# jdeschut/tunempc

Hardware: AMD Instinct MI355X
Metric: stage-Hessian convexifications/sec at (nx+nu)=32, p=64 (higher is better)
Workload: dtype f64

## Files before the change

### include/tunempc_hip.h

```cpp
#ifndef TUNEMPC_HIP_H
#define TUNEMPC_HIP_H

#include <stdint.h>

#ifdef __cplusplus
extern "C" {
#endif

#define TMPC_OK 0
#define TMPC_E_ARG (-1)
#define TMPC_E_UNSUPPORTED (-2)
#define TMPC_E_NOMEM (-3)
#define TMPC_E_HIP (-4)
#define TMPC_E_NODEVICE (-5)
#define TMPC_E_NOCONV (-6)

#define TMPC_STATUS_OPTIMAL 0
#define TMPC_STATUS_FEASIBLE 1
#define TMPC_STATUS_INFEASIBLE 2

#define TMPC_FLAG_NO_MFMA 1
#define TMPC_FLAG_PROFILE 2
#define TMPC_FLAG_FAST_EXIT 4

// ... 15 lines not shown
int tmpc_destroy(tmpc_handle* h);
int tmpc_get_chunk(tmpc_handle* h);

int tmpc_set_options(tmpc_handle* h, double tol, double center_tol, int max_iter, int center_iter, int flags);

#define TMPC_TUNE_CHORD_STEP 1
#define TMPC_TUNE_SMALL_BLOCKS 2
#define TMPC_TUNE_EIG_PRETEST 3
#define TMPC_TUNE_FUSE_FWD 4
#define TMPC_TUNE_GRAPH 5
#define TMPC_TUNE_PERSISTENT 7
#define TMPC_TUNE_LOWP_SWITCH 8
#define TMPC_LOWP_SWITCH_DEFAULT 1e-5
#define TMPC_TUNE_LOWP_TRSM 9
#define TMPC_TUNE_TRSM_PAIR 10
int tmpc_set_tuning(tmpc_handle* h, int key, double value);
int tmpc_create_ex(tmpc_handle** out, int chunk, int p, int nx, int mb, int ng, int nc, int step3, int lanes);

int tmpc_set_tight(tmpc_handle* h, int enable, double tight_tol);

int tmpc_convexify_batch_host(tmpc_handle* h, int nb, const double* A, const double* B, const double* H,
                              double* Hc, double* dHc, double* P, double* alpha, double* beta, double* kappa,
                              int32_t* status, int32_t* iters, double* info);
int tmpc_convexify_batch_device(tmpc_handle* h, int nb, const double* dA, const double* dB, const double* dH,
                                double* dHc_out, double* ddHc_out, double* dP_out, double* d_alpha, double* d_beta,
                                double* d_kappa, int32_t* d_status, int32_t* d_iters, double* d_info, void* stream);

int tmpc_convexify_eq_batch_host(tmpc_handle* h, int nb, const double* A, const double* B, const double* H, const double* G,
                                 double* Hc, double* dHc, double* P, double* Fg, double* alpha, double* beta, double* kappa,
                                 int32_t* status, int32_t* iters, double* info);
// ... 167 lines not shown
```

### include/tunempc_hip_debug.h

```cpp
#ifndef TUNEMPC_HIP_DEBUG_H
#define TUNEMPC_HIP_DEBUG_H

#include "tunempc_hip.h"

#ifdef __cplusplus
extern "C" {
#endif

#define TMPC_DEBUG_FLAG_STOP_ASSEMBLED 8
#define TMPC_DEBUG_FLAG_NO_LIFT 16
#define TMPC_DEBUG_FLAG_NO_DMA 32
#define TMPC_DEBUG_FLAG_GENERIC_STAGE 64

int tmpc_debug_gemm_nt(tmpc_handle* h, double* C, const double* A, const double* B, int M, int N, int K, int mode, int lower);

int tmpc_debug_block_solve(tmpc_handle* h, int p, int d, const double* D, const double* Ccpl, const double* rhs, double* x, int32_t* nshift);

#define TMPC_DEBUG_FACTOR_PASS1 1
#define TMPC_DEBUG_FACTOR_FUSE_FWD1 2
#define TMPC_DEBUG_FACTOR_LOWP_TRSM 4
#define TMPC_DEBUG_FACTOR_DD 8
typedef struct {
  const double *D, *Ccpl, *Dlo, *Clo, *rhs;
  const int32_t *list, *lowp;
  double *oD, *oO, *oF, *oDdiag, *oX;
  float* oO32;
  double *oDl, *oOl, *oFl, *oXl;
  int32_t *nshift, *dims, *orient;
} tmpc_debug_factor_io;
int tmpc_debug_block_factor(tmpc_handle* h, int nb, int p, int d, int count, int mode, const tmpc_debug_factor_io* io);
long long tmpc_debug_last_trsm_pairs(void);

int tmpc_debug_cr_schedule(int p, int32_t* out, int cap);

int tmpc_debug_get_multipliers(tmpc_handle* h, int nb, int nr, double* phi, double* z, double* dphi, double* dz);

int tmpc_debug_get_array(tmpc_handle* h, int which, uint64_t offset, uint64_t count, double* out);

int tmpc_debug_set_stop_iteration(tmpc_handle* h, int k);

int tmpc_debug_min_eig(tmpc_handle* h, int nmat, int n, const double* W, double* out);
int tmpc_debug_min_eig_lane(tmpc_handle* h, int nmat, int n, const double* W, double* out);

int tmpc_debug_factor_bench(tmpc_handle* h, int nb, int p, int d, int reps, double* ms_out2);

#ifdef __cplusplus
// ... 4 lines not shown
```

### tunempc_amd/_lib.py

```python
import ctypes as C
import os

import numpy as np

_HERE = os.path.dirname(os.path.abspath(__file__))
_LIB = None

INFO_STRIDE = 16
FLAG_NO_MFMA = 1
FLAG_PROFILE = 2
FLAG_FAST_EXIT = 4
STATUS_NAMES = {0: 'Optimal', 1: 'Feasible', 2: 'Infeasible'}

ARROW_LD = 32
EXPORTS = [
    'tmpc_device_count', 'tmpc_workspace_bytes', 'tmpc_workspace_bytes_eq', 'tmpc_workspace_bytes_con',
    'tmpc_create', 'tmpc_create_eq', 'tmpc_create_con', 'tmpc_destroy', 'tmpc_get_chunk', 'tmpc_set_options', 'tmpc_set_tight', 'tmpc_set_tuning', 'tmpc_create_ex',
    'tmpc_convexify_batch_host', 'tmpc_convexify_batch_device', 'tmpc_convexify_eq_batch_host', 'tmpc_convexify_step2_batch_host',
    'tmpc_convexify_con_batch_device', 'tmpc_workspace_bytes_step3', 'tmpc_create_step3', 'tmpc_convexify_step3_batch_host', 'tmpc_workspace_bytes_step3_con', 'tmpc_create_step3_con', 'tmpc_convexify_step3_con_batch_host', 'tmpc_convexify_step3_batch_device', 'tmpc_convexify_step3_con_batch_device', 'tmpc_supplement_batch_host', 'tmpc_supplement_terms_batch_host',
    'tmpc_tracking_reference_host', 'tmpc_eig_scan_host', 'tmpc_get_profile', 'tmpc_get_trace', 'tmpc_get_dual_host', 'tmpc_get_dual_con_host', 'tmpc_pack_sensitivities_host', 'tmpc_eig_clip_host',
    'tmpc_periodic_lqr_batch_host', 'tmpc_periodic_lqr_batch_device', 'tmpc_periodic_lqr_rows_batch_host', 'tmpc_periodic_lqr_rows_batch_device',
    'tmpc_periodic_lqr_ctg_batch_host', 'tmpc_periodic_lqr_ctg_batch_device', 'tmpc_horizon_lqr_batch_host', 'tmpc_horizon_lqr_batch_device',
    'tmpc_closed_loop_batch_host', 'tmpc_closed_loop_batch_device', 'tmpc_mpc_qp_batch_host', 'tmpc_mpc_qp_batch_device',
    'tmpc_mpc_qp_soft_batch_host', 'tmpc_mpc_qp_soft_batch_device', 'tmpc_mpc_qp_eq_batch_host', 'tmpc_mpc_qp_eq_batch_device',
    'tmpc_mpc_qp_aff_batch_host', 'tmpc_mpc_qp_aff_batch_device', 'tmpc_mpc_qp_quad_batch_host', 'tmpc_mpc_qp_quad_batch_device',
    'tmpc_mpc_qp_warm_batch_host', 'tmpc_mpc_qp_warm_batch_device',
    'tmpc_last_error', 'tmpc_version',
]
DEBUG_EXPORTS = [
    'tmpc_debug_gemm_nt', 'tmpc_debug_block_solve', 'tmpc_debug_cr_schedule', 'tmpc_debug_get_multipliers', 'tmpc_debug_get_array',
    'tmpc_debug_min_eig', 'tmpc_debug_min_eig_lane', 'tmpc_debug_factor_bench', 'tmpc_debug_block_factor',
    'tmpc_debug_last_trsm_pairs', 'tmpc_debug_set_stop_iteration',
]
FLAG_DEBUG_NO_DMA = 32
FACTOR_PASS1, FACTOR_FUSE_FWD1, FACTOR_LOWP_TRSM, FACTOR_DD = 1, 2, 4, 8


class _FactorIO(C.Structure):
    _fields_ = ([(n, C.POINTER(C.c_double)) for n in ('D', 'Ccpl', 'Dlo', 'Clo', 'rhs')] + [(n, C.POINTER(C.c_int32)) for n in ('list', 'lowp')] +
                [(n, C.POINTER(C.c_double)) for n in ('oD', 'oO', 'oF', 'oDdiag', 'oX')] + [('oO32', C.POINTER(C.c_float))] +
                [(n, C.POINTER(C.c_double)) for n in ('oDl', 'oOl', 'oFl', 'oXl')] + [(n, C.POINTER(C.c_int32)) for n in ('nshift', 'dims', 'orient')])


def library_path():
    return os.environ.get('TMPC_LIB') or os.path.join(_HERE, 'lib', 'libtunempc_hip.so')


# ... 131 lines not shown
    lib.tmpc_debug_gemm_nt.argtypes = [vp, dp, dp, dp, C.c_int, C.c_int, C.c_int, C.c_int, C.c_int]
    lib.tmpc_debug_block_solve.restype = C.c_int
    lib.tmpc_debug_block_solve.argtypes = [vp, C.c_int, C.c_int, dp, dp, dp, dp, ip]
    lib.tmpc_supplement_terms_batch_host.restype = C.c_int
    lib.tmpc_supplement_terms_batch_host.argtypes = [vp, C.c_int, dp, dp, dp, C.c_int, dp, dp, dp, dp]
    lib.tmpc_tracking_reference_host.restype = C.c_int
    lib.tmpc_tracking_reference_host.argtypes = [vp, C.c_int, dp, dp, dp, C.c_double, dp, dp, ip]
    lib.tmpc_debug_cr_schedule.restype = C.c_int
    lib.tmpc_debug_cr_schedule.argtypes = [C.c_int, ip, C.c_int]
    lib.tmpc_debug_block_factor.restype = C.c_int
    lib.tmpc_debug_block_factor.argtypes = [vp, C.c_int, C.c_int, C.c_int, C.c_int, C.c_int, C.POINTER(_FactorIO)]
    lib.tmpc_debug_factor_bench.restype = C.c_int
    lib.tmpc_debug_factor_bench.argtypes = [vp, C.c_int, C.c_int, C.c_int, C.c_int, dp]
    lib.tmpc_debug_last_trsm_pairs.restype = C.c_longlong
    lib.tmpc_debug_last_trsm_pairs.argtypes = []
    lib.tmpc_debug_min_eig.restype = C.c_int
    lib.tmpc_debug_min_eig.argtypes = [vp, C.c_int, C.c_int, dp, dp]
    lib.tmpc_debug_min_eig_lane.restype = C.c_int
    lib.tmpc_debug_min_eig_lane.argtypes = [vp, C.c_int, C.c_int, dp, dp]
    lib.tmpc_last_error.restype = C.c_char_p
    lib.tmpc_version.restype = C.c_char_p
    _LIB = lib
    return lib


def _dptr(a):
    return a.ctypes.data_as(C.POINTER(C.c_double)) if a is not None else None


def _iptr(a):
# ... 34 lines not shown
            _check(self.lib, self.lib.tmpc_create_step3_con(C.byref(self._h), int(chunk), self.p, self.nx, self.mb, self.ng, self.nc), 'tmpc_create_step3_con')
        elif self.step3:
            _check(self.lib, self.lib.tmpc_create_step3(C.byref(self._h), int(chunk), self.p, self.nx, self.mb), 'tmpc_create_step3')
        else:
            _check(self.lib, self.lib.tmpc_create_con(C.byref(self._h), int(chunk), self.p, self.nx, self.mb, self.ng, self.nc), 'tmpc_create_con')
        self.chunk = int(self.lib.tmpc_get_chunk(self._h))
        self.flags = int(flags)
        self.set_options(tol, center_tol, max_iter, center_iter, flags)

    def set_options(self, tol=None, center_tol=None, max_iter=None, center_iter=None, flags=None):
        if flags is not None:
            self.flags = int(flags)
        _check(self.lib, self.lib.tmpc_set_options(self._h, float(tol or 0.0), float(center_tol or 0.0),
                                                   int(max_iter or 0), int(center_iter or 0), self.flags), 'tmpc_set_options')

    def set_tuning(self, chord_step=None, small_blocks=None, eig_pretest=None, fuse_fwd=None, graph=None, persistent=None, lowp_switch=None, lowp_trsm=None, trsm_pair=None):
        for key, v in ((1, chord_step), (2, small_blocks), (3, eig_pretest), (4, fuse_fwd), (5, graph), (7, persistent), (8, lowp_switch), (9, lowp_trsm), (10, trsm_pair)):
            if v is not None:
                _check(self.lib, self.lib.tmpc_set_tuning(self._h, key, float(v)), 'tmpc_set_tuning')

    def set_tight(self, enable=True, tight_tol=None):
        _check(self.lib, self.lib.tmpc_set_tight(self._h, 1 if enable else 0, float(tight_tol or 0.0)), 'tmpc_set_tight')

    def close(self):
        if getattr(self, '_h', None) is not None and self._h.value:
            self.lib.tmpc_destroy(self._h)
            self._h = C.c_void_p()

    def __del__(self):
        try:
            self.close()
        except Exception:
# ... 283 lines not shown
        if Hc.shape[-2:] != (n, n) or q.shape != Hc.shape[:-1] or wref.shape != q.shape:
            raise ValueError('tracking_reference: expected Hc [..., %d, %d] and q, wref [..., %d]' % (n, n, n))
        ns = int(np.prod(Hc.shape[:-2], dtype=np.int64))
        W = np.empty_like(Hc); yref = np.empty_like(q); info = np.zeros(Hc.shape[:-2], dtype=np.int32)
        _check(self.lib, self.lib.tmpc_tracking_reference_host(self._h, ns, _dptr(Hc), _dptr(q), _dptr(wref), float(ts), _dptr(W), _dptr(yref),
                                                              info.ctypes.data_as(C.POINTER(C.c_int32))), 'tmpc_tracking_reference_host')
        return W, yref, info

    def debug_factor_bench(self, nb, p, d, reps=3):
        out = np.zeros(2)
        _check(self.lib, self.lib.tmpc_debug_factor_bench(self._h, nb, p, d, reps, _dptr(out)), 'tmpc_debug_factor_bench')
        return out

    def debug_last_trsm_pairs(self):
        return int(self.lib.tmpc_debug_last_trsm_pairs())

    def debug_block_solve(self, D, Ccpl, rhs):
        D = np.ascontiguousarray(D, dtype=np.float64); Ccpl = np.ascontiguousarray(Ccpl, dtype=np.float64)
        rhs = np.ascontiguousarray(rhs, dtype=np.float64)
        p, d, _ = D.shape
        x = np.empty((p, d)); ns = np.zeros(1, np.int32)
        _check(self.lib, self.lib.tmpc_debug_block_solve(self._h, p, d, _dptr(D), _dptr(Ccpl), _dptr(rhs), _dptr(x), _iptr(ns)), 'tmpc_debug_block_solve')
        return x, int(ns[0])

    def debug_block_factor(self, D, Ccpl, rhs, plist=None, lowp=None, pass1=False, fuse_fwd1=False, lowp_trsm=False, dd=False, Dlo=None, Clo=None):
        f64 = lambda a: None if a is None else np.ascontiguousarray(a, dtype=np.float64)
        D, Ccpl, rhs, Dlo, Clo = f64(D), f64(Ccpl), f64(rhs), f64(Dlo), f64(Clo)
        nb, p, d, _ = D.shape
        nc = 3 if pass1 else 1
        if Ccpl.shape != D.shape or rhs.shape != ((nb, p, d, 3) if pass1 else (nb, p, d)):
# ... 430 lines not shown
```

### tunempc_amd/csrc/tmpc_api.hip

```cpp
#include <hip/hip_runtime.h>
#include <stdio.h>
#include <stdlib.h>
#include <new>
#include <string.h>
#include <algorithm>
#include <chrono>
#include <thread>
#include <mutex>
#include <condition_variable>
#include <functional>
#include <unistd.h>
#include <vector>

#include <string>
#include <unordered_map>

#include "../../include/tunempc_hip.h"
#include "../../include/tunempc_hip_debug.h"
#include "tmpc_common.h"
#include "tmpc_small.h"
#include "tmpc_stage.h"
#include "tmpc_schur.h"
#include "tmpc_factor.h"
#include "tmpc_cr.h"
// ... 96 lines not shown
struct tmpc_handle {
  Dims dm;
  int chunk;
  int nlanes;
  Opts opt;
  int flags;
  int stop_it;
  Lane lane[MAXL];
  void* slab;
  size_t slab_bytes;
  hipEvent_t ev_in;
  int device;
  CrSched sched;
  int* d_sched;
  int rs, mt;
  int tune_small, tune_pretest, tune_fuse, tune_graph, tune_persist, tune_lowp_trsm, tune_trsm_pair;
  void* dd_slab;
  size_t dd_bytes;
  int tight;
  double tight_tol;
};

static int cr_upload(const CrSched& sc, int** out) {
  std::vector<int> flat(sc.elim);
  flat.insert(flat.end(), sc.upd.begin(), sc.upd.end());
  flat.insert(flat.end(), sc.orient.begin(), sc.orient.end());
  *out = nullptr;
  if (hipMalloc(out, flat.size() * sizeof(int)) != hipSuccess) return TMPC_E_NOMEM;
  if (hipMemcpy(*out, flat.data(), flat.size() * sizeof(int), hipMemcpyHostToDevice) != hipSuccess) { hipFree(*out); *out = nullptr; return TMPC_E_HIP; }
  return TMPC_OK;
}
// ... 274 lines not shown
  const int m0 = 64 * tm, n0 = 64 * tn;
  const int Mt = M - m0 < 64 ? M - m0 : 64, Nt = N - n0 < 64 ? N - n0 : 64;
  const double* A0 = A + (size_t)m0 * K; const double* B0 = B + (size_t)n0 * K;
  if (k1 > 0 && k1 < K && 2 * k1 == K)
    wg_tile_dma<UPD_DMA_DEPTH>(C + (size_t)m0 * N + n0, N, A0, B0, A0 + k1, B0 + k1, K, Mt, Nt, k1, mode, (lower && tm == tn) ? 0 : GM_NOTRI, blockIdx.x, lds);
  else
    wg_tile_dma<UPD_DMA_DEPTH>(C + (size_t)m0 * N + n0, N, A0, B0, nullptr, nullptr, K, Mt, Nt, K, mode, (lower && tm == tn) ? 0 : GM_NOTRI, blockIdx.x, lds);
}
static size_t slots_bytes(int s) { return (size_t)s * MS * sizeof(double); }
template <int PART> static size_t schur_lds(const Dims& dm) {
  if (!schur_in_lds(dm)) return (size_t)dm.d * sizeof(unsigned) + 64;
 return (size_t)sch_rec<PART>() * dm.nx * dm.nx * sizeof(double) + (size_t)dm.d * sizeof(unsigned) + 64; }
static size_t factor_lds() { return (size_t)FACT_LDS_DOUBLES * sizeof(double); }
static size_t solve_lds(const Dims& dm) { return (size_t)cr_solve_lds_doubles(dm.dp) * sizeof(double); }

static int set_lds_attrs(int device) {
  static bool done[64] = {false};
  if (device >= 0 && device < 64 && done[device]) return TMPC_OK;
  const int big = 160 * 1024;
  HIPCHK(hipFuncSetAttribute((const void*)k_stage_pre<256>, hipFuncAttributeMaxDynamicSharedMemorySize, big - 4096));
  HIPCHK(hipFuncSetAttribute((const void*)k_stage_rhs<256>, hipFuncAttributeMaxDynamicSharedMemorySize, big - 4096));
  HIPCHK(hipFuncSetAttribute((const void*)k_stage_dir<256>, hipFuncAttributeMaxDynamicSharedMemorySize, big - 4096));
  HIPCHK(hipFuncSetAttribute((const void*)k_final_stage, hipFuncAttributeMaxDynamicSharedMemorySize, big));
  HIPCHK(hipFuncSetAttribute((const void*)k_schur<0>, hipFuncAttributeMaxDynamicSharedMemorySize, big));
  HIPCHK(hipFuncSetAttribute((const void*)k_schur<1>, hipFuncAttributeMaxDynamicSharedMemorySize, big));
  HIPCHK(hipFuncSetAttribute((const void*)k_cr_potrf<true>, hipFuncAttributeMaxDynamicSharedMemorySize, big));
  HIPCHK(hipFuncSetAttribute((const void*)k_cr_potrf<false>, hipFuncAttributeMaxDynamicSharedMemorySize, big));
  HIPCHK(hipFuncSetAttribute((const void*)k_cr_trsm<true, 2>, hipFuncAttributeMaxDynamicSharedMemorySize, big));
  HIPCHK(hipFuncSetAttribute((const void*)k_cr_trsm<false, 2>, hipFuncAttributeMaxDynamicSharedMemorySize, big));
  HIPCHK(hipFuncSetAttribute((const void*)k_cr_trsm_dma, hipFuncAttributeMaxDynamicSharedMemorySize, big));
  HIPCHK(hipFuncSetAttribute((const void*)k_cr_trsm_dma_f32, hipFuncAttributeMaxDynamicSharedMemorySize, big));
  HIPCHK(hipFuncSetAttribute((const void*)k_cr_potrf_dma, hipFuncAttributeMaxDynamicSharedMemorySize, big));
  HIPCHK(hipFuncSetAttribute((const void*)k_cr_update<true, 2>, hipFuncAttributeMaxDynamicSharedMemorySize, big));
  HIPCHK(hipFuncSetAttribute((const void*)k_cr_update<false, 2>, hipFuncAttributeMaxDynamicSharedMemorySize, big));
  HIPCHK(hipFuncSetAttribute((const void*)k_cr_fwd_diag, hipFuncAttributeMaxDynamicSharedMemorySize, big));
  HIPCHK(hipFuncSetAttribute((const void*)k_cr_fwd_off, hipFuncAttributeMaxDynamicSharedMemorySize, big));
  HIPCHK(hipFuncSetAttribute((const void*)k_cr_bwd, hipFuncAttributeMaxDynamicSharedMemorySize, big));
  HIPCHK(hipFuncSetAttribute((const void*)k_cr_small_solve, hipFuncAttributeMaxDynamicSharedMemorySize, big));
  HIPCHK(hipFuncSetAttribute((const void*)k_cr_small_factor, hipFuncAttributeMaxDynamicSharedMemorySize, big));
  HIPCHK(hipFuncSetAttribute((const void*)k_ipm_small, hipFuncAttributeMaxDynamicSharedMemorySize, big));
// ... 265 lines not shown
    }
  }
  auto ipm_loop = [&](const Opts& o, bool ddm, int cap) -> int {
  while (active > 0 && it < cap) {
    const int BP = active * dm.p;
    hipGraphExec_t gexec = nullptr;
    std::string gkey;
    bool capturing = false;
    struct CaptureGuard {
      hipStream_t st; bool* on;
      ~CaptureGuard() { if (*on) { hipGraph_t g_ = nullptr; (void)hipStreamEndCapture(st, &g_); if (g_) hipGraphDestroy(g_); (void)hipGetLastError(); } }
    } capture_guard{st, &capturing};
    int nkev = 0;
    if (use_graph && !ddm) {
      gkey.assign((const char*)&w, sizeof(WS)); gkey.append((const char*)&dm, sizeof(Dims)); gkey.append((const char*)&o, sizeof(Opts));
      const int ks[6] = {active, nfac, nb, reg_max, (int)h->flags, h->tune_pretest | (h->tune_fuse << 1) | (h->tune_small << 2)};
      gkey.append((const char*)ks, sizeof(ks));
      if (!ln->graphs) ln->graphs = new std::unordered_map<std::string, hipGraphExec_t>();
      auto f = ln->graphs->find(gkey);
      if (f == ln->graphs->end()) {
        if (ln->graphs->size() >= 256) { for (auto& kv : *ln->graphs) if (kv.second) hipGraphExecDestroy(kv.second); ln->graphs->clear(); }
        (*ln->graphs)[gkey] = nullptr;
      } else if (f->second) gexec = f->second;
      else if (hipStreamBeginCapture(st, hipStreamCaptureModeThreadLocal) == hipSuccess) capturing = true;
    }
    if (!gexec) {
    if (prof) HIPCHK(hipEventRecord(ln->ev[0], st));
    if (big) hipLaunchKernelGGL(kb_stage_pre, dim3(BP), dim3(256), 0, st, w, dm);
    else TMPC_STAGE_LAUNCH(k_stage_pre, slots_bytes(PRE_SLOTS), st, w, dm);
    if (eq) {
      const bool bigr = dm.nr > NRS;
      if (big && bigr) hipLaunchKernelGGL((k_phi_pre<true, true>), dim3(BP), dim3(64), (size_t)phi_pre_lds(true, true) * sizeof(double), st, w, dm, 1);
      else if (big) hipLaunchKernelGGL((k_phi_pre<true, false>), dim3(BP), dim3(64), (size_t)phi_pre_lds(true, false) * sizeof(double), st, w, dm, 1);
      else if (bigr) hipLaunchKernelGGL((k_phi_pre<false, true>), dim3(BP), dim3(64), (size_t)phi_pre_lds(false, true) * sizeof(double), st, w, dm, 1);
      else hipLaunchKernelGGL((k_phi_pre<false, false>), dim3(BP), dim3(64), (size_t)phi_pre_lds(false, false) * sizeof(double), st, w, dm, 1);
    }
    if (t3) hipLaunchKernelGGL(k_t3_pre, dim3(BP), dim3(64), t3_lds, st, w, dm);
    hipLaunchKernelGGL(k_ctrl_a, dim3(active), dim3(64), 0, st, w, dm, o);
    if (prof) HIPCHK(hipEventRecord(ln->ev[1], st));
    if (ddm) {
      if (nfac > 0) {
        hipLaunchKernelGGL(k_dd_images, dim3(nfac * dm.p), dim3(256), dd_stage_lds(dm, DD_IMG_SLOTS), st, wf, dm);
        dd_schur_launch(wf, dm, nfac * dm.p, st);
      }
    } else if (nfac > 0) {
      if (schur_in_lds(dm)) {
        hipLaunchKernelGGL(k_schur<0>, dim3(nfac * dm.p), dim3(SCH_NT), schur_lds<0>(dm), st, wf, dm);
        hipLaunchKernelGGL(k_schur<1>, dim3(nfac * dm.p), dim3(SCH_NT), schur_lds<1>(dm), st, wf, dm);
      } else {
        hipLaunchKernelGGL((k_schur<0, true>), dim3(nfac * dm.p), dim3(SCH_NT), schur_lds<0>(dm), st, wf, dm);
        hipLaunchKernelGGL((k_schur<1, true>), dim3(nfac * dm.p), dim3(SCH_NT), schur_lds<1>(dm), st, wf, dm);
      }
    }
    if (eq && nfac > 0 && ddm) hipLaunchKernelGGL(k_dd_aug_fill, dim3(nfac * dm.p), dim3(256), (size_t)dd_aug_lds_doubles(dm.nr, dm.n, dm.nx) * sizeof(double), st, wf, dm, 0);
    else if (eq && nfac > 0) hipLaunchKernelGGL(k_aug_fill, dim3(nfac * dm.p), dim3(64), 0, st, wf, dm);
    if (t3 && nfac > 0 && big) hipLaunchKernelGGL(k_t3_schur<true>, dim3(nfac * dm.p), dim3(256), t3_schur_lds, st, wf, dm);
    else if (t3 && nfac > 0) hipLaunchKernelGGL(k_t3_schur<false>, dim3(nfac * dm.p), dim3(256), t3_schur_lds, st, wf, dm);
    if (t3 && eq && nfac > 0) hipLaunchKernelGGL(k_t3_cross, dim3(nfac * dm.p), dim3(64), 0, st, wf, dm);
    if ((h->flags & TMPC_DEBUG_FLAG_STOP_ASSEMBLED) && it + 1 >= h->stop_it) {
      if (big) hipLaunchKernelGGL(kb_stage_rhs, dim3(BP), dim3(256), 0, st, w, dm, 1);
      else TMPC_STAGE_LAUNCH(k_stage_rhs, slots_bytes(RHS_SLOTS), st, w, dm, 1);
      if (t3) hipLaunchKernelGGL(k_t3_rhs, dim3(BP), dim3(64), t3_lds, st, w, dm, 1);
      hipLaunchKernelGGL(k_gather, dim3(BP), dim3(64), 0, st, w, dm, 1);
      if (t3) hipLaunchKernelGGL(k_t3_gather, dim3(BP), dim3(64), 0, st, w, dm, 1);
      HIPCHK(hipStreamSynchronize(st));
// ... 238 lines not shown
  }
  tmpc_handle* h = new (std::nothrow) tmpc_handle();
  if (!h) return TMPC_E_NOMEM;
  h->slab = nullptr; h->d_sched = nullptr; h->ev_in = nullptr; h->dd_slab = nullptr; h->dd_bytes = 0; h->tight = 0; h->tight_tol = 0x1p-37;
  if (hipGetDevice(&h->device) != hipSuccess) { delete h; return TMPC_E_HIP; }
  int nl = (make_dims(1, p, nx, mb, ng, nc, step3).dp <= 64 && chunk >= 2) ? 2 : 1;
  if (lanes >= 1) nl = std::min(lanes, MAXL);
  nl = std::max(1, std::min(nl, chunk));
  h->nlanes = nl;
  const int cap = (chunk + nl - 1) / nl;
  h->chunk = cap * nl;
  h->dm = make_dims(cap, p, nx, mb, ng, nc, step3);
  h->sched = cr_build(p);
  h->rs = 0; h->mt = 0;
  h->tune_small = 1; h->tune_pretest = 1; h->tune_fuse = 1; h->tune_graph = 1; h->tune_persist = 1; h->tune_lowp_trsm = 1; h->tune_trsm_pair = 1;
  h->opt.tol = 0x1p-25; h->opt.center_tol = 1e-9; h->opt.max_iter = 50; h->opt.center_iter = 12;
  h->opt.fast_exit = 0;
  h->opt.lowp_switch = TMPC_LOWP_SWITCH_DEFAULT;
  h->opt.chord_step = 10.0;
  h->flags = 0; h->stop_it = 1;
  WS tmp;
  const size_t lane_bytes = carve(tmp, h->dm, nullptr, nullptr);
  h->slab_bytes = lane_bytes * nl;
  if (hipMalloc(&h->slab, h->slab_bytes) != hipSuccess) {
    snprintf(g_err, sizeof(g_err), "hipMalloc(%zu bytes) failed", h->slab_bytes);
    delete h;
    return TMPC_E_NOMEM;
  }
  int rc = cr_upload(h->sched, &h->d_sched);
  bool ok = (rc == TMPC_OK) && hipEventCreateWithFlags(&h->ev_in, hipEventDisableTiming) == hipSuccess;
// ... 52 lines not shown
}


int tmpc_set_tuning(tmpc_handle* h, int key, double value) {
  if (!h) return TMPC_E_ARG;
  switch (key) {
    case TMPC_TUNE_CHORD_STEP: if (!(value >= 0.0)) return TMPC_E_ARG; h->opt.chord_step = value; return TMPC_OK;
    case TMPC_TUNE_LOWP_SWITCH: if (!(value >= 0.0)) return TMPC_E_ARG; h->opt.lowp_switch = value; return TMPC_OK;
    case TMPC_TUNE_SMALL_BLOCKS: h->tune_small = value != 0.0; return TMPC_OK;
    case TMPC_TUNE_EIG_PRETEST: h->tune_pretest = value != 0.0; return TMPC_OK;
    case TMPC_TUNE_FUSE_FWD: h->tune_fuse = value != 0.0; return TMPC_OK;
    case TMPC_TUNE_GRAPH: h->tune_graph = value != 0.0; return TMPC_OK;
    case TMPC_TUNE_PERSISTENT: if (!(value >= 0.0 && value <= 2.0)) return TMPC_E_ARG; h->tune_persist = (int)value; return TMPC_OK;
    case TMPC_TUNE_LOWP_TRSM: h->tune_lowp_trsm = value != 0.0; return TMPC_OK;
    case TMPC_TUNE_TRSM_PAIR: h->tune_trsm_pair = value != 0.0; return TMPC_OK;
    default: snprintf(g_err, sizeof(g_err), "tmpc_set_tuning: unknown key %d", key); return TMPC_E_ARG;
  }
}

int tmpc_set_tight(tmpc_handle* h, int enable, double tight_tol) {
  if (!h) return TMPC_E_ARG;
  if (!enable) { h->tight = 0; return TMPC_OK; }
  if (h->dm.nT > 0) { snprintf(g_err, sizeof(g_err), "tmpc_set_tight: Steps 1 and 2 only (no Step 3 handles)"); return TMPC_E_UNSUPPORTED; }
  if (h->dm.nr > 0 && (size_t)dd_aug_lds_doubles(h->dm.nr, h->dm.n, h->dm.nx) * sizeof(double) > 160 * 1024) {
    snprintf(g_err, sizeof(g_err), "tmpc_set_tight: %d rows per stage at nx = %d, nx + mb = %d: their double-double vectors do not fit the LDS (rows * (2 n + 2 nx) <= 4040)", h->dm.nr, h->dm.nx, h->dm.n);
    return TMPC_E_UNSUPPORTED;
  }
  if ((size_t)dd_solve_lds_doubles(h->dm.dp) * sizeof(double) > 160 * 1024) {
    snprintf(g_err, sizeof(g_err), "tmpc_set_tight: Schur blocks of %d do not fit the LDS image of the double-double substitution kernels (nx <= 51)", h->dm.dp);
    return TMPC_E_UNSUPPORTED;
// ... 1463 lines not shown
  HIPCHK(hipMemcpy(cb.w.Z, hz.data(), (size_t)p * dp * 8, hipMemcpyHostToDevice));
  cr_factor(cb.w, cb.dm, cb.sc, cb.d_sched, cb.w.alist, 1, 0, h->rs, h->mt, nullptr, nullptr, 0, cb.w.O32 ? 1 : 0);
  cr_solve(cb.w, cb.dm, cb.sc, cb.d_sched, cb.w.alist, 1, 0, 2);
  HIPCHK(hipDeviceSynchronize());
  HIPCHK(hipGetLastError());
  int hip_[IS];
  HIPCHK(hipMemcpy(hz.data(), cb.w.Z, (size_t)p * dp * 8, hipMemcpyDeviceToHost));
  HIPCHK(hipMemcpy(hip_, cb.w.iprob, sizeof(hip_), hipMemcpyDeviceToHost));
  for (int k = 0; k < p; ++k) for (int i = 0; i < d; ++i) x[(size_t)k * d + i] = hz[(size_t)k * dp + i];
  if (nshift) *nshift = hip_[I_NSHIFT];
  return TMPC_OK;
}

static long long g_last_trsm_pairs = 0;
long long tmpc_debug_last_trsm_pairs(void) { return g_last_trsm_pairs; }
int tmpc_debug_block_factor(tmpc_handle* h, int nb, int p, int d, int count, int mode, const tmpc_debug_factor_io* io) {
  if (!h || !io || nb < 1 || p < 1 || d < 1 || count < 0 || count > nb || !io->D || !io->Ccpl || !io->rhs || (count > 0 && !io->list)) return TMPC_E_ARG;
  if (mode & ~(TMPC_DEBUG_FACTOR_PASS1 | TMPC_DEBUG_FACTOR_FUSE_FWD1 | TMPC_DEBUG_FACTOR_LOWP_TRSM | TMPC_DEBUG_FACTOR_DD)) return TMPC_E_ARG;
  const bool pass1 = (mode & TMPC_DEBUG_FACTOR_PASS1) != 0, fuse = (mode & TMPC_DEBUG_FACTOR_FUSE_FWD1) != 0, ddm = (mode & TMPC_DEBUG_FACTOR_DD) != 0;
  std::vector<char> seen(nb, 0);
  int nlowp = 0, anylowp = 0;
  for (int i = 0; i < count; ++i) {
    const int b = io->list[i];
    if (b < 0 || b >= nb || seen[b]) { snprintf(g_err, sizeof(g_err), "tmpc_debug_block_factor: list entry %d is out of range or repeated", i); return TMPC_E_ARG; }
    seen[b] = 1;
    if (io->lowp && io->lowp[b]) ++nlowp;
  }
  for (int b = 0; b < nb && io->lowp; ++b) anylowp |= io->lowp[b] != 0;
  ON_DEVICE(h);
  CrBench cb;
// ... 164 lines not shown
```

### tunempc_amd/csrc/tmpc_schur.h

```cpp
#pragma once
#include "tmpc_common.h"
#include "tmpc_small.h"

namespace tmpc {

#ifndef TMPC_POLISH_ENTER
#define TMPC_POLISH_ENTER 1e-4
#endif
constexpr double POLISH_ENTER_GPU = TMPC_POLISH_ENTER;
constexpr int MUT_BACKOFF_MAX = 10;

constexpr int SCH_NT = 320;
template <int PART> constexpr int sch_rec() { return PART == 0 ? 10 : 6; }
__device__ __forceinline__ double hkm_t(double xac, double xad, double xbc, double xbd, double sac, double sad, double sbc, double sbd) {
  return (xac * sbd + xad * sbc) + (xbc * sad + xbd * sac);
}
template <int PART, bool GF, int NTS>
__device__ __forceinline__ void schur_body(const WS& w, const Dims& dm, int sid, int tid, double* sm) {
  constexpr int REC = sch_rec<PART>();
  const int b = sid / dm.p, k = sid - b * dm.p;
  const int* ip = w.iprob + (size_t)b * IS;
  if (ip[I_PHASE] == PH_DONE) return;
  const int nx = dm.nx, nxx = nx * nx, d = dm.d, dp = dm.dp;
  const int reg = ip[I_REG];
  const double regf = (reg <= 0) ? 1.0 : 1.0 + 1e-13 * ((reg == 1) ? 10.0 : (reg == 2) ? 100.0 : 1000.0);
  double* mats = GF ? w.sscr + (size_t)sid * 10 * nxx : sm;
  unsigned* pair = (unsigned*)(GF ? sm : sm + (size_t)nxx * REC);
  const bool corner = (w.cr_orient[k] != 0);
  const int km = (k == 0) ? dm.p - 1 : k - 1;
  const double* kfk = w.KF + (size_t)sid * 12 * nxx;
  const double* kfm = w.KF + (size_t)(b * dm.p + km) * 12 * nxx;
  for (int e = tid; e < 12 * nxx; e += NTS) {
// ... 4 lines not shown
    const double v = (slot == KF_KX || slot == KF_KS) ? kfm[e] : kfk[e];
    int i = r / nx, j = r - i * nx;
    if (fmat && !corner) { const int t_ = i; i = j; j = t_; }
    const int q = fmat ? 2 * lmi + (slot - KF_FX) : 4 * lmi + slot;
    mats[(size_t)(i * nx + j) * REC + q] = v;
  }
  if (tid < nx) {
    int e = tid * nx - (tid * (tid - 1)) / 2;
    for (int c = tid; c < nx; ++c) pair[e++] = (unsigned)tid | ((unsigned)c << 16);
  }
  if (NTS == 64) asm volatile("s_waitcnt vmcnt(0) lgkmcnt(0)" ::: "memory");
  else __syncthreads();
  double* Dg = w.D + (size_t)sid * dp * dp;
  double* Cg = w.O + (size_t)sid * dp * dp;
  double* dd = w.Ddiag + (size_t)sid * dp;
  for (int col = tid; col < dp; col += NTS) {
    const bool cin = col < d;
    const unsigned pc_ = cin ? pair[col] : 0u;
    const int c = (int)(pc_ & 0xffffu), d_ = (int)(pc_ >> 16);
    const double wc = (c == d_) ? 0.5 : 1.0;
    const double2_t* rc = (const double2_t*)(mats + (size_t)c * REC);
    const double2_t* rd = (const double2_t*)(mats + (size_t)d_ * REC);
    constexpr int NQ = PART == 0 ? 4 : 2;
    double2_t ac[NQ], ad[NQ];
    int a_prev = -1;
    const int row0 = (PART == 0) ? (col / 64) * 64 : 0;
    for (int row = row0; row < dp; ++row) {
      const size_t e = (size_t)row * dp + col;
      if (row >= d || !cin) {
        if (PART == 0) { if (col <= row) Dg[e] = (row == col) ? 1.0 : 0.0; if (row == col) dd[row] = 1.0; }
        else Cg[e] = 0.0;
        continue;
      }
      const unsigned pr_ = (unsigned)__builtin_amdgcn_readfirstlane((int)pair[row]);
      const int a = (int)(pr_ & 0xffffu), bb = (int)(pr_ >> 16);
      const int ro = nx * (REC / 2);
      if (a != a_prev) {
        a_prev = a;
#pragma unroll
        for (int q = 0; q < NQ; ++q) { ac[q] = rc[a * ro + q]; ad[q] = rd[a * ro + q]; }
      }
      const double wgt = ((a == bb) ? 0.5 : 1.0) * wc;
      if (PART == 1) {
        const double2_t bc0 = rc[bb * ro], bd0 = rd[bb * ro], bc1 = rc[bb * ro + 1], bd1 = rd[bb * ro + 1];
        double cv = 0.0;
        cv -= wgt * hkm_t(ac[0][0], ad[0][0], bc0[0], bd0[0], ac[0][1], ad[0][1], bc0[1], bd0[1]);
        cv -= wgt * hkm_t(ac[1][0], ad[1][0], bc1[0], bd1[0], ac[1][1], ad[1][1], bc1[1], bd1[1]);
        Cg[e] = cv;
      } else if (col <= row) {
        double dv = 0.0;
#pragma unroll
        for (int r = 0; r < 2; ++r) {
          const double2_t bc0 = rc[bb * ro + 2 * r], bd0 = rd[bb * ro + 2 * r];
          const double2_t bc1 = rc[bb * ro + 2 * r + 1], bd1 = rd[bb * ro + 2 * r + 1];
          dv += wgt * hkm_t(ac[2 * r][0], ad[2 * r][0], bc0[0], bd0[0], ac[2 * r][1], ad[2 * r][1], bc0[1], bd0[1]);
          dv += wgt * hkm_t(ac[2 * r + 1][0], ad[2 * r + 1][0], bc1[0], bd1[0], ac[2 * r + 1][1], ad[2 * r + 1][1], bc1[1], bd1[1]);
        }
        if (row == col) { dv *= regf; dd[row] = dv; }
        Dg[e] = dv;
      }
    }
  }
}

template <int PART, bool GF = false>
__global__ void __launch_bounds__(SCH_NT) k_schur(WS w, Dims dm) {
  extern __shared__ __attribute__((aligned(16))) double sm[];
  schur_body<PART, GF, SCH_NT>(w, dm, stage_id(w, dm), threadIdx.x, sm);
}

__device__ __forceinline__ void gather_body(const WS& w, const Dims& dm, int sid, int lane, int pass) {
  const int b = sid / dm.p, k = sid - b * dm.p;
  const int* ip = w.iprob + (size_t)b * IS;
  const int phase = ip[I_PHASE];
  if (phase == PH_DONE) return;
  if (pass == 1 && phase != PH_MAIN) return;
  const bool three = (pass == 1) || (phase != PH_MAIN && !ip[I_CHORD]);
  const int nx = dm.nx, nxx = nx * nx, dp = dm.dp;
  const int km = (k == 0) ? dm.p - 1 : k - 1;
  const double* av = w.adjV + (size_t)(b * dm.p + km) * NADJ * nxx;
  const double* ae = w.adjE + (size_t)sid * NADJ * nxx;
  int e = 0;
  for (int a = 0; a < nx; ++a) {
// ... 295 lines not shown
```

Measured before the change: 12840.

## Balance Schur D-block work across waves with a flattened row walk

Adds a walk mode for the D part of the Schur kernel. The lower-triangular rows of each 64-column group are flattened into one item list, and each wave takes an equal contiguous slice of it, using a configurable wave count (5, 8 or 10, default 8). Before, each thread owned whole columns, and column groups with more rows made some waves run much longer than others. The cost is more kernel instantiations, and each wave's column coefficients are reloaded at slice boundaries.

```diff
diff --git a/include/tunempc_hip.h b/include/tunempc_hip.h
--- a/include/tunempc_hip.h
+++ b/include/tunempc_hip.h
@@ -53,6 +53,13 @@
 #define TMPC_LOWP_SWITCH_DEFAULT 1e-5
 #define TMPC_TUNE_LOWP_TRSM 9
 #define TMPC_TUNE_TRSM_PAIR 10
+#define TMPC_TUNE_SCHUR_WALK 11
+#ifndef TMPC_SCHUR_WALK_DEFAULT
+#define TMPC_SCHUR_WALK_DEFAULT 1
+#endif
+#ifndef TMPC_SCHUR_WALK_DEFAULT_NW
+#define TMPC_SCHUR_WALK_DEFAULT_NW 8
+#endif
 int tmpc_set_tuning(tmpc_handle* h, int key, double value);
 int tmpc_create_ex(tmpc_handle** out, int chunk, int p, int nx, int mb, int ng, int nc, int step3, int lanes);
 
diff --git a/include/tunempc_hip_debug.h b/include/tunempc_hip_debug.h
--- a/include/tunempc_hip_debug.h
+++ b/include/tunempc_hip_debug.h
@@ -30,6 +30,7 @@
 } tmpc_debug_factor_io;
 int tmpc_debug_block_factor(tmpc_handle* h, int nb, int p, int d, int count, int mode, const tmpc_debug_factor_io* io);
 long long tmpc_debug_last_trsm_pairs(void);
+int tmpc_debug_last_schur_waves(void);
 
 int tmpc_debug_cr_schedule(int p, int32_t* out, int cap);
 
diff --git a/tunempc_amd/_lib.py b/tunempc_amd/_lib.py
--- a/tunempc_amd/_lib.py
+++ b/tunempc_amd/_lib.py
@@ -30,7 +30,7 @@
 DEBUG_EXPORTS = [
     'tmpc_debug_gemm_nt', 'tmpc_debug_block_solve', 'tmpc_debug_cr_schedule', 'tmpc_debug_get_multipliers', 'tmpc_debug_get_array',
     'tmpc_debug_min_eig', 'tmpc_debug_min_eig_lane', 'tmpc_debug_factor_bench', 'tmpc_debug_block_factor',
-    'tmpc_debug_last_trsm_pairs', 'tmpc_debug_set_stop_iteration',
+    'tmpc_debug_last_trsm_pairs', 'tmpc_debug_last_schur_waves', 'tmpc_debug_set_stop_iteration',
 ]
 FLAG_DEBUG_NO_DMA = 32
 FACTOR_PASS1, FACTOR_FUSE_FWD1, FACTOR_LOWP_TRSM, FACTOR_DD = 1, 2, 4, 8
@@ -192,6 +192,8 @@
     lib.tmpc_debug_factor_bench.argtypes = [vp, C.c_int, C.c_int, C.c_int, C.c_int, dp]
     lib.tmpc_debug_last_trsm_pairs.restype = C.c_longlong
     lib.tmpc_debug_last_trsm_pairs.argtypes = []
+    lib.tmpc_debug_last_schur_waves.restype = C.c_int
+    lib.tmpc_debug_last_schur_waves.argtypes = []
     lib.tmpc_debug_min_eig.restype = C.c_int
     lib.tmpc_debug_min_eig.argtypes = [vp, C.c_int, C.c_int, dp, dp]
     lib.tmpc_debug_min_eig_lane.restype = C.c_int
@@ -256,8 +258,8 @@
         _check(self.lib, self.lib.tmpc_set_options(self._h, float(tol or 0.0), float(center_tol or 0.0),
                                                    int(max_iter or 0), int(center_iter or 0), self.flags), 'tmpc_set_options')
 
-    def set_tuning(self, chord_step=None, small_blocks=None, eig_pretest=None, fuse_fwd=None, graph=None, persistent=None, lowp_switch=None, lowp_trsm=None, trsm_pair=None):
-        for key, v in ((1, chord_step), (2, small_blocks), (3, eig_pretest), (4, fuse_fwd), (5, graph), (7, persistent), (8, lowp_switch), (9, lowp_trsm), (10, trsm_pair)):
+    def set_tuning(self, chord_step=None, small_blocks=None, eig_pretest=None, fuse_fwd=None, graph=None, persistent=None, lowp_switch=None, schur_walk=None, lowp_trsm=None, trsm_pair=None):
+        for key, v in ((1, chord_step), (2, small_blocks), (3, eig_pretest), (4, fuse_fwd), (5, graph), (7, persistent), (8, lowp_switch), (9, lowp_trsm), (10, trsm_pair), (11, schur_walk)):
             if v is not None:
                 _check(self.lib, self.lib.tmpc_set_tuning(self._h, key, float(v)), 'tmpc_set_tuning')
 
@@ -571,6 +573,9 @@
 
     def debug_last_trsm_pairs(self):
         return int(self.lib.tmpc_debug_last_trsm_pairs())
+
+    def debug_last_schur_waves(self):
+        return int(self.lib.tmpc_debug_last_schur_waves())
 
     def debug_block_solve(self, D, Ccpl, rhs):
         D = np.ascontiguousarray(D, dtype=np.float64); Ccpl = np.ascontiguousarray(Ccpl, dtype=np.float64)
diff --git a/tunempc_amd/csrc/tmpc_api.hip b/tunempc_amd/csrc/tmpc_api.hip
--- a/tunempc_amd/csrc/tmpc_api.hip
+++ b/tunempc_amd/csrc/tmpc_api.hip
@@ -134,7 +134,7 @@
   CrSched sched;
   int* d_sched;
   int rs, mt;
-  int tune_small, tune_pretest, tune_fuse, tune_graph, tune_persist, tune_lowp_trsm, tune_trsm_pair;
+  int tune_small, tune_pretest, tune_fuse, tune_graph, tune_persist, tune_lowp_trsm, tune_trsm_pair, tune_schur_walk;
   void* dd_slab;
   size_t dd_bytes;
   int tight;
@@ -439,6 +439,14 @@
 static size_t factor_lds() { return (size_t)FACT_LDS_DOUBLES * sizeof(double); }
 static size_t solve_lds(const Dims& dm) { return (size_t)cr_solve_lds_doubles(dm.dp) * sizeof(double); }
 
+static int g_last_schur_waves = 0;
+template <bool GF> static void schur_d_launch(int walk_nw, int grid, size_t lds, hipStream_t st, const WS& wf, const Dims& dm) {
+  if (walk_nw == 5) hipLaunchKernelGGL((k_schur<0, GF, 5, true>), dim3(grid), dim3(320), lds, st, wf, dm);
+  else if (walk_nw == 8) hipLaunchKernelGGL((k_schur<0, GF, 8, true>), dim3(grid), dim3(512), lds, st, wf, dm);
+  else if (walk_nw == 10) hipLaunchKernelGGL((k_schur<0, GF, 10, true>), dim3(grid), dim3(640), lds, st, wf, dm);
+  else hipLaunchKernelGGL((k_schur<0, GF>), dim3(grid), dim3(SCH_NT), lds, st, wf, dm);
+}
+
 static int set_lds_attrs(int device) {
   static bool done[64] = {false};
   if (device >= 0 && device < 64 && done[device]) return TMPC_OK;
@@ -449,6 +457,9 @@
   HIPCHK(hipFuncSetAttribute((const void*)k_final_stage, hipFuncAttributeMaxDynamicSharedMemorySize, big));
   HIPCHK(hipFuncSetAttribute((const void*)k_schur<0>, hipFuncAttributeMaxDynamicSharedMemorySize, big));
   HIPCHK(hipFuncSetAttribute((const void*)k_schur<1>, hipFuncAttributeMaxDynamicSharedMemorySize, big));
+  HIPCHK(hipFuncSetAttribute((const void*)k_schur<0, false, 5, true>, hipFuncAttributeMaxDynamicSharedMemorySize, big));
+  HIPCHK(hipFuncSetAttribute((const void*)k_schur<0, false, 8, true>, hipFuncAttributeMaxDynamicSharedMemorySize, big));
+  HIPCHK(hipFuncSetAttribute((const void*)k_schur<0, false, 10, true>, hipFuncAttributeMaxDynamicSharedMemorySize, big));
   HIPCHK(hipFuncSetAttribute((const void*)k_cr_potrf<true>, hipFuncAttributeMaxDynamicSharedMemorySize, big));
   HIPCHK(hipFuncSetAttribute((const void*)k_cr_potrf<false>, hipFuncAttributeMaxDynamicSharedMemorySize, big));
   HIPCHK(hipFuncSetAttribute((const void*)k_cr_trsm<true, 2>, hipFuncAttributeMaxDynamicSharedMemorySize, big));
@@ -744,7 +755,7 @@
     int nkev = 0;
     if (use_graph && !ddm) {
       gkey.assign((const char*)&w, sizeof(WS)); gkey.append((const char*)&dm, sizeof(Dims)); gkey.append((const char*)&o, sizeof(Opts));
-      const int ks[6] = {active, nfac, nb, reg_max, (int)h->flags, h->tune_pretest | (h->tune_fuse << 1) | (h->tune_small << 2)};
+      const int ks[6] = {active, nfac, nb, reg_max, (int)h->flags, h->tune_pretest | (h->tune_fuse << 1) | (h->tune_small << 2) | (h->tune_schur_walk << 3)};
       gkey.append((const char*)ks, sizeof(ks));
       if (!ln->graphs) ln->graphs = new std::unordered_map<std::string, hipGraphExec_t>();
       auto f = ln->graphs->find(gkey);
@@ -754,6 +765,7 @@
       } else if (f->second) gexec = f->second;
       else if (hipStreamBeginCapture(st, hipStreamCaptureModeThreadLocal) == hipSuccess) capturing = true;
     }
+    if (!ddm && nfac > 0) g_last_schur_waves = h->tune_schur_walk ? h->tune_schur_walk : SCH_NT / 64;
     if (!gexec) {
     if (prof) HIPCHK(hipEventRecord(ln->ev[0], st));
     if (big) hipLaunchKernelGGL(kb_stage_pre, dim3(BP), dim3(256), 0, st, w, dm);
@@ -775,10 +787,10 @@
       }
     } else if (nfac > 0) {
       if (schur_in_lds(dm)) {
-        hipLaunchKernelGGL(k_schur<0>, dim3(nfac * dm.p), dim3(SCH_NT), schur_lds<0>(dm), st, wf, dm);
+        schur_d_launch<false>(h->tune_schur_walk, nfac * dm.p, schur_lds<0>(dm), st, wf, dm);
         hipLaunchKernelGGL(k_schur<1>, dim3(nfac * dm.p), dim3(SCH_NT), schur_lds<1>(dm), st, wf, dm);
       } else {
-        hipLaunchKernelGGL((k_schur<0, true>), dim3(nfac * dm.p), dim3(SCH_NT), schur_lds<0>(dm), st, wf, dm);
+        schur_d_launch<true>(h->tune_schur_walk, nfac * dm.p, schur_lds<0>(dm), st, wf, dm);
         hipLaunchKernelGGL((k_schur<1, true>), dim3(nfac * dm.p), dim3(SCH_NT), schur_lds<1>(dm), st, wf, dm);
       }
     }
@@ -1047,6 +1059,7 @@
   h->sched = cr_build(p);
   h->rs = 0; h->mt = 0;
   h->tune_small = 1; h->tune_pretest = 1; h->tune_fuse = 1; h->tune_graph = 1; h->tune_persist = 1; h->tune_lowp_trsm = 1; h->tune_trsm_pair = 1;
+  h->tune_schur_walk = TMPC_SCHUR_WALK_DEFAULT == 1 ? TMPC_SCHUR_WALK_DEFAULT_NW : TMPC_SCHUR_WALK_DEFAULT;
   h->opt.tol = 0x1p-25; h->opt.center_tol = 1e-9; h->opt.max_iter = 50; h->opt.center_iter = 12;
   h->opt.fast_exit = 0;
   h->opt.lowp_switch = TMPC_LOWP_SWITCH_DEFAULT;
@@ -1129,6 +1142,9 @@
     case TMPC_TUNE_PERSISTENT: if (!(value >= 0.0 && value <= 2.0)) return TMPC_E_ARG; h->tune_persist = (int)value; return TMPC_OK;
     case TMPC_TUNE_LOWP_TRSM: h->tune_lowp_trsm = value != 0.0; return TMPC_OK;
     case TMPC_TUNE_TRSM_PAIR: h->tune_trsm_pair = value != 0.0; return TMPC_OK;
+    case TMPC_TUNE_SCHUR_WALK:
+      if (!(value == 0.0 || value == 1.0 || value == 5.0 || value == 8.0 || value == 10.0)) return TMPC_E_ARG;
+      h->tune_schur_walk = value == 1.0 ? TMPC_SCHUR_WALK_DEFAULT_NW : (int)value; return TMPC_OK;
     default: snprintf(g_err, sizeof(g_err), "tmpc_set_tuning: unknown key %d", key); return TMPC_E_ARG;
   }
 }
@@ -2622,6 +2638,7 @@
 
 static long long g_last_trsm_pairs = 0;
 long long tmpc_debug_last_trsm_pairs(void) { return g_last_trsm_pairs; }
+int tmpc_debug_last_schur_waves(void) { return g_last_schur_waves; }
 int tmpc_debug_block_factor(tmpc_handle* h, int nb, int p, int d, int count, int mode, const tmpc_debug_factor_io* io) {
   if (!h || !io || nb < 1 || p < 1 || d < 1 || count < 0 || count > nb || !io->D || !io->Ccpl || !io->rhs || (count > 0 && !io->list)) return TMPC_E_ARG;
   if (mode & ~(TMPC_DEBUG_FACTOR_PASS1 | TMPC_DEBUG_FACTOR_FUSE_FWD1 | TMPC_DEBUG_FACTOR_LOWP_TRSM | TMPC_DEBUG_FACTOR_DD)) return TMPC_E_ARG;
diff --git a/tunempc_amd/csrc/tmpc_schur.h b/tunempc_amd/csrc/tmpc_schur.h
--- a/tunempc_amd/csrc/tmpc_schur.h
+++ b/tunempc_amd/csrc/tmpc_schur.h
@@ -15,7 +15,65 @@
 __device__ __forceinline__ double hkm_t(double xac, double xad, double xbc, double xbd, double sac, double sad, double sbc, double sbd) {
   return (xac * sbd + xad * sbc) + (xbc * sad + xbd * sac);
 }
-template <int PART, bool GF, int NTS>
+__host__ __device__ __forceinline__ int sch_walk_items(int dp) {
+  int t = 0;
+  for (int g0 = 0; g0 < dp; g0 += 64) t += dp - g0;
+  return t;
+}
+__host__ __device__ __forceinline__ void sch_walk_chunk(int dp, int nw, int wave, int* lo, int* hi) {
+  const long long t = sch_walk_items(dp);
+  *lo = (int)(wave * t / nw); *hi = (int)((wave + 1) * t / nw);
+}
+template <int PART>
+__device__ __forceinline__ void schur_col_rows(const double* mats, const unsigned* pair, double* Dg, double* Cg, double* dd, int nx, int d, int dp, double regf,
+                                               int col, int rbeg, int rend) {
+  constexpr int REC = sch_rec<PART>();
+  const bool cin = col < d;
+  const unsigned pc_ = cin ? pair[col] : 0u;
+  const int c = (int)(pc_ & 0xffffu), d_ = (int)(pc_ >> 16);
+  const double wc = (c == d_) ? 0.5 : 1.0;
+  const double2_t* rc = (const double2_t*)(mats + (size_t)c * REC);
+  const double2_t* rd = (const double2_t*)(mats + (size_t)d_ * REC);
+  constexpr int NQ = PART == 0 ? 4 : 2;
+  double2_t ac[NQ], ad[NQ];
+  int a_prev = -1;
+  for (int row = rbeg; row < rend; ++row) {
+    const size_t e = (size_t)row * dp + col;
+    if (row >= d || !cin) {
+      if (PART == 0) { if (col <= row) Dg[e] = (row == col) ? 1.0 : 0.0; if (row == col) dd[row] = 1.0; }
+      else Cg[e] = 0.0;
+      continue;
+    }
+    const unsigned pr_ = (unsigned)__builtin_amdgcn_readfirstlane((int)pair[row]);
+    const int a = (int)(pr_ & 0xffffu), bb = (int)(pr_ >> 16);
+    const int ro = nx * (REC / 2);
+    if (a != a_prev) {
+      a_prev = a;
+#pragma unroll
+      for (int q = 0; q < NQ; ++q) { ac[q] = rc[a * ro + q]; ad[q] = rd[a * ro + q]; }
+    }
+    const double wgt = ((a == bb) ? 0.5 : 1.0) * wc;
+    if (PART == 1) {
+      const double2_t bc0 = rc[bb * ro], bd0 = rd[bb * ro], bc1 = rc[bb * ro + 1], bd1 = rd[bb * ro + 1];
+      double cv = 0.0;
+      cv -= wgt * hkm_t(ac[0][0], ad[0][0], bc0[0], bd0[0], ac[0][1], ad[0][1], bc0[1], bd0[1]);
+      cv -= wgt * hkm_t(ac[1][0], ad[1][0], bc1[0], bd1[0], ac[1][1], ad[1][1], bc1[1], bd1[1]);
+      Cg[e] = cv;
+    } else if (col <= row) {
+      double dv = 0.0;
+#pragma unroll
+      for (int r = 0; r < 2; ++r) {
+        const double2_t bc0 = rc[bb * ro + 2 * r], bd0 = rd[bb * ro + 2 * r];
+        const double2_t bc1 = rc[bb * ro + 2 * r + 1], bd1 = rd[bb * ro + 2 * r + 1];
+        dv += wgt * hkm_t(ac[2 * r][0], ad[2 * r][0], bc0[0], bd0[0], ac[2 * r][1], ad[2 * r][1], bc0[1], bd0[1]);
+        dv += wgt * hkm_t(ac[2 * r + 1][0], ad[2 * r + 1][0], bc1[0], bd1[0], ac[2 * r + 1][1], ad[2 * r + 1][1], bc1[1], bd1[1]);
+      }
+      if (row == col) { dv *= regf; dd[row] = dv; }
+      Dg[e] = dv;
+    }
+  }
+}
+template <int PART, bool GF, int NTS, bool WALK = false>
 __device__ __forceinline__ void schur_body(const WS& w, const Dims& dm, int sid, int tid, double* sm) {
   constexpr int REC = sch_rec<PART>();
   const int b = sid / dm.p, k = sid - b * dm.p;
@@ -50,59 +108,30 @@
   double* Dg = w.D + (size_t)sid * dp * dp;
   double* Cg = w.O + (size_t)sid * dp * dp;
   double* dd = w.Ddiag + (size_t)sid * dp;
+  if (PART == 0 && WALK) {
+    const int wave = __builtin_amdgcn_readfirstlane(tid >> 6), lane = tid & 63;
+    int lo, hi;
+    sch_walk_chunk(dp, NTS / 64, wave, &lo, &hi);
+    int g0 = 0;
+    while (lo >= dp - g0) { lo -= dp - g0; hi -= dp - g0; g0 += 64; }
+    for (int row = g0 + lo, n = hi - lo; n > 0; g0 += 64, row = g0) {
+      const int rend = (row + n < dp) ? row + n : dp;
+      if (g0 + lane < dp) schur_col_rows<PART>(mats, pair, Dg, Cg, dd, nx, d, dp, regf, g0 + lane, row, rend);
+      n -= rend - row;
+    }
+    return;
+  }
   for (int col = tid; col < dp; col += NTS) {
-    const bool cin = col < d;
-    const unsigned pc_ = cin ? pair[col] : 0u;
-    const int c = (int)(pc_ & 0xffffu), d_ = (int)(pc_ >> 16);
-    const double wc = (c == d_) ? 0.5 : 1.0;
-    const double2_t* rc = (const double2_t*)(mats + (size_t)c * REC);
-    const double2_t* rd = (const double2_t*)(mats + (size_t)d_ * REC);
-    constexpr int NQ = PART == 0 ? 4 : 2;
-    double2_t ac[NQ], ad[NQ];
-    int a_prev = -1;
     const int row0 = (PART == 0) ? (col / 64) * 64 : 0;
-    for (int row = row0; row < dp; ++row) {
-      const size_t e = (size_t)row * dp + col;
-      if (row >= d || !cin) {
-        if (PART == 0) { if (col <= row) Dg[e] = (row == col) ? 1.0 : 0.0; if (row == col) dd[row] = 1.0; }
-        else Cg[e] = 0.0;
-        continue;
-      }
-      const unsigned pr_ = (unsigned)__builtin_amdgcn_readfirstlane((int)pair[row]);
-      const int a = (int)(pr_ & 0xffffu), bb = (int)(pr_ >> 16);
-      const int ro = nx * (REC / 2);
-      if (a != a_prev) {
-        a_prev = a;
-#pragma unroll
-        for (int q = 0; q < NQ; ++q) { ac[q] = rc[a * ro + q]; ad[q] = rd[a * ro + q]; }
-      }
-      const double wgt = ((a == bb) ? 0.5 : 1.0) * wc;
-      if (PART == 1) {
-        const double2_t bc0 = rc[bb * ro], bd0 = rd[bb * ro], bc1 = rc[bb * ro + 1], bd1 = rd[bb * ro + 1];
-        double cv = 0.0;
-        cv -= wgt * hkm_t(ac[0][0], ad[0][0], bc0[0], bd0[0], ac[0][1], ad[0][1], bc0[1], bd0[1]);
-        cv -= wgt * hkm_t(ac[1][0], ad[1][0], bc1[0], bd1[0], ac[1][1], ad[1][1], bc1[1], bd1[1]);
-        Cg[e] = cv;
-      } else if (col <= row) {
-        double dv = 0.0;
-#pragma unroll
-        for (int r = 0; r < 2; ++r) {
-          const double2_t bc0 = rc[bb * ro + 2 * r], bd0 = rd[bb * ro + 2 * r];
-          const double2_t bc1 = rc[bb * ro + 2 * r + 1], bd1 = rd[bb * ro + 2 * r + 1];
-          dv += wgt * hkm_t(ac[2 * r][0], ad[2 * r][0], bc0[0], bd0[0], ac[2 * r][1], ad[2 * r][1], bc0[1], bd0[1]);
-          dv += wgt * hkm_t(ac[2 * r + 1][0], ad[2 * r + 1][0], bc1[0], bd1[0], ac[2 * r + 1][1], ad[2 * r + 1][1], bc1[1], bd1[1]);
-        }
-        if (row == col) { dv *= regf; dd[row] = dv; }
-        Dg[e] = dv;
-      }
-    }
-  }
-}
-
-template <int PART, bool GF = false>
-__global__ void __launch_bounds__(SCH_NT) k_schur(WS w, Dims dm) {
+    schur_col_rows<PART>(mats, pair, Dg, Cg, dd, nx, d, dp, regf, col, row0, dp);
+  }
+}
+
+template <int PART, bool GF = false, int NW = SCH_NT / 64, bool WALK = false>
+__global__ void __launch_bounds__(64 * NW) k_schur(WS w, Dims dm) {
+  static_assert(!WALK || PART == 0, "the flattened walk is the D part's");
   extern __shared__ __attribute__((aligned(16))) double sm[];
-  schur_body<PART, GF, SCH_NT>(w, dm, stage_id(w, dm), threadIdx.x, sm);
+  schur_body<PART, GF, 64 * NW, WALK>(w, dm, stage_id(w, dm), threadIdx.x, sm);
 }
 
 __device__ __forceinline__ void gather_body(const WS& w, const Dims& dm, int sid, int lane, int pass) {
```

After: 12930 (median of 6 runs). About the same (+0.7%).
